# pingcap/tidb

Measured on NVIDIA H100. Metric: hash-join probe rows/sec, higher is better.
Workload: dtype int64

## Files before the change

tidb_b200/csrc/join.cu:

```cuda
#include <memory>
#include <deque>
#include <algorithm>
#include <cmath>
#include <condition_variable>
#include "join_kernels.cuh"
#include "partition_kernels.cuh"
#include "chunk_io.cuh"

namespace tg {

static const int64_t kGeneralBatchRows = 16ll << 20;
static const int64_t kDirectPushRows = 128ll << 10;
static const int64_t kNextWindowRows = 1ll << 20;

struct Side {
  int ncols = 0;
  std::vector<int> types;
  std::vector<uint32_t> flags;
  std::vector<int> elem;
  std::vector<int> kelem;
  bool has_cells = false;
  std::vector<char> needed;
  int key_col = -1;
  std::vector<int> key_cols;
// ... 664 lines not shown
  for (int c : j->build.used) if (j->build.kelem[c] != 8 || j->bcols.has_nulls[c]) return false;
  for (int e : j->kout_elem) if (e != 8) return false;
  return true;
}

static bool build_fast_out(const JoinImpl* j, const OutCols& oc, const DevCols& pview, FastOut& fo) {
  std::memset(&fo, 0, sizeof(fo));
  int pcol_of[TG_FAST_MAX_PCOLS];
  for (int c = 0; c < oc.n; c++) {
    const OutSpec& sp = oc.spec[c];
    unsigned long long* dst = reinterpret_cast<unsigned long long*>(oc.data[c]);
    if (sp.src == SRC_BUILD_KEY || (sp.src == SRC_PROBE_COL && sp.idx == j->probe.key_col)) {
      if (fo.n_key_dst >= TG_FAST_MAX_KEYDST) return false;
      fo.key_dst[fo.n_key_dst++] = dst;
    } else if (sp.src == SRC_BUILD_META) {
      if (fo.n_meta_dst >= TG_FAST_MAX_METADST) return false;
      fo.meta_dst[fo.n_meta_dst++] = dst;
    } else if (sp.src == SRC_PROBE_COL) {
      for (int q = 0; q < fo.n_pcols; q++) if (pcol_of[q] == sp.idx) return false;
      if (fo.n_pcols >= TG_FAST_MAX_PCOLS) return false;
      int k = fo.n_pcols++;
      pcol_of[k] = sp.idx;
      fo.psrc[k] = reinterpret_cast<const unsigned long long*>(pview.data[sp.idx]);
      fo.pdst[k] = dst;
    } else return false;
  }
  return true;
}

template <template <int, int, int> class F, typename... A>
static int dispatch_shape(const FastOut& fo, A&&... a) {
#define TG_SHAPE(P, K, M) if (fo.n_pcols == P && fo.n_key_dst == K && fo.n_meta_dst == M) return F<P, K, M>::run(a...);
#define TG_SHAPE_KM(P) TG_SHAPE(P, 0, 0) TG_SHAPE(P, 0, 1) TG_SHAPE(P, 1, 0) TG_SHAPE(P, 1, 1) TG_SHAPE(P, 2, 0) TG_SHAPE(P, 2, 1)
  TG_SHAPE_KM(0) TG_SHAPE_KM(1) TG_SHAPE_KM(2) TG_SHAPE_KM(3)
#undef TG_SHAPE_KM
#undef TG_SHAPE
  return fail(TG_ERR_CUDA, "internal: fused probe shape not instantiated");
}

template <int NPC, int NKD, int NMD>
struct LaunchWarp {
  static int run(JoinImpl* j, const int64_t* pkey, int64_t n, const FastOut& fo, unsigned long long* cur, const ProbeTuning& t, const SegSpec& seg) {
    constexpr int R = 4;
    static int resident = 0;
    if (!resident) {
      int nb = 0;
      if (cudaOccupancyMaxActiveBlocksPerMultiprocessor(&nb, k_probe_inner_u1_w<R, NPC, NKD, NMD>, 256, 0) != cudaSuccess || nb < 1) { cudaGetLastError(); nb = 3; }
      resident = nb;
      if (getenv("TG_DEBUG")) fprintf(stderr, "[tidbgpu] k_probe_inner_u1_w<%d,%d,%d>: %d resident CTAs per SM\n", NPC, NKD, NMD, nb);
    }
    int64_t tiles = (n + 32 * R - 1) / (32 * R);
    int64_t ctas = (tiles + 7) / 8;
    int per_sm = t.ctas_per_sm > 0 ? t.ctas_per_sm : resident;
    int grid = (int)std::min<int64_t>(ctas, (int64_t)j->nsm * per_sm);
    k_probe_inner_u1_w<R, NPC, NKD, NMD><<<grid, 256, 0, j->stream>>>(pkey, n, j->tv, fo, cur, seg);
    return TG_OK;
  }
};
template <int NPC, int NKD, int NMD>
struct LaunchSeg {
  static int run(JoinImpl* j, const int64_t* pkey, int64_t n, const FastOut& fo, unsigned long long* cur, const ProbeTuning& t, const SegSpec& seg) {
    static int resident = 0;
    if (!resident) {
      int nb = 0;
      if (cudaOccupancyMaxActiveBlocksPerMultiprocessor(&nb, k_probe_inner_u1_seg_lean<NPC, NKD, NMD>, 256, 0) != cudaSuccess || nb < 1) { cudaGetLastError(); nb = 3; }
      resident = nb;
    }
    int64_t ctas = (n / 128 + 7) / 8;
    int per_sm = t.ctas_per_sm > 0 ? t.ctas_per_sm : resident;
    int grid = (int)std::min<int64_t>(ctas, (int64_t)j->nsm * per_sm);
    k_probe_inner_u1_seg_lean<NPC, NKD, NMD><<<grid, 256, 0, j->stream>>>(pkey, n, j->tv, fo, cur, seg);
    return TG_OK;
  }
};
template <int NPC, int NKD, int NMD>
struct LaunchInplace {
  static int run(JoinImpl* j, int64_t n, const FastOut& fo, unsigned long long* cur, const ProbeTuning& t, const SegSpec& seg, uint32_t* tile_cnt) {
    if constexpr (NKD == 0) {
      return fail(TG_ERR_CUDA, "internal: the in-place segment probe needs an output fed by the join key");
    } else {
      static int resident = 0;
      if (!resident) {
        int nb = 0;
        if (cudaOccupancyMaxActiveBlocksPerMultiprocessor(&nb, k_probe_inner_u1_seg_inplace<NPC, NKD, NMD>, 256, 0) != cudaSuccess || nb < 1) { cudaGetLastError(); nb = 3; }
        resident = nb;
      }
      int64_t ctas = (n / 128 + 7) / 8;
      int per_sm = t.ctas_per_sm > 0 ? t.ctas_per_sm : resident;
      int grid = (int)std::min<int64_t>(ctas, (int64_t)j->nsm * per_sm);
      k_probe_inner_u1_seg_inplace<NPC, NKD, NMD><<<grid, 256, 0, j->stream>>>(n, j->tv, fo, cur, seg, tile_cnt);
      return TG_OK;
    }
  }
};
static int launch_probe_warp(JoinImpl* j, const int64_t* pkey, int64_t n, const FastOut& fo, unsigned long long* cur, const ProbeTuning& t,
                             const SegSpec& seg = SegSpec{nullptr, 0, 0, 0, nullptr}) {
  j->stats.paths |= TG_JOIN_PATH_PROBE_DIRECT;
  return dispatch_shape<LaunchWarp>(fo, j, pkey, n, fo, cur, t, seg);
}
static int launch_probe_seg(JoinImpl* j, const int64_t* pkey, int64_t n, const FastOut& fo, unsigned long long* cur, const ProbeTuning& t, const SegSpec& seg) {
  j->stats.paths |= TG_JOIN_PATH_PROBE_SEG;
  return dispatch_shape<LaunchSeg>(fo, j, pkey, n, fo, cur, t, seg);
}
static bool aligned16(const void* p) { return (reinterpret_cast<uintptr_t>(p) & 15) == 0; }

static int probe_device(JoinImpl* j, const DevCols& pcells, int64_t n, ResultBatch& rb, bool sync_count, const SegSpec* in_seg = nullptr) {
  const Side& p = j->probe;
  DevCols pview = pcells;
  TG_TRY(kernel_view(j, p, pview, n));
  j->stats.probe_rows += n;
  KeySpec ks = j->probe_key;
  if (j->multi_key) {
    if (in_seg) return fail(TG_ERR_UNSUPPORTED, "segmented device chunks: joins on several key columns take the general path");
    TG_TRY(composite_key(j, p, pview, n, j->pkey_syn, j->pkey_syn_nn));
    ks.data = j->pkey_syn.p; ks.nulls = j->pkey_syn_nn.as<uint8_t>();
  } else { ks.data = pview.data[p.key_col]; ks.nulls = pview.nulls[p.key_col]; }
  TG_TRY(j->out_cursor.ensure(j->device, 64));
  OutCols oc{};
  fill_outspec_probe(j, oc);
  FastOut fo{};
  const bool fast = fast_path_ok(j, pview) && build_fast_out(j, oc, pview, fo);
  if (in_seg && !fast) return fail(TG_ERR_UNSUPPORTED, "segmented device chunks are only accepted by the fused fast path (unique build keys, <= 1 payload, no filters, an output shape the warp kernels cover)");
  if (fast) {
    const ProbeTuning& tune = probe_tuning();
    const int64_t* pkey = reinterpret_cast<const int64_t*>(ks.data);
    const size_t table_bytes = (size_t)j->tv.nslots * sizeof(Slot);
    bool src16 = aligned16(pkey);
    for (int c = 0; c < fo.n_pcols; c++) src16 = src16 && aligned16(fo.psrc[c]);
    const int64_t PTILE = 1024;
    const int64_t n_main = n / PTILE * PTILE;
    int P = 0;
    int64_t C = 0;
    if (n > 0 && tune.partition && src16 && n >= (int64_t)tune.part_min_rows && table_bytes > ((size_t)tune.part_min_mb << 20)) {
      P = probe_slices(table_bytes, j->device, tune.parts);
      C = ((int64_t)((double)n_main / P * 1.05) + 16384 + 127) / 128 * 128;
      if (!(P >= 2 && (int64_t)P * C / 128 < (1ll << 31))) P = 0;
    }
    const bool inplace = P && !in_seg && rb.rows == 0 && fo.n_key_dst >= 1 &&
                         (tune.inplace >= 0 ? tune.inplace != 0 : j->seg_match >= kInplaceMinMatch);
    if (inplace) C = inplace_seg_cap(j, P, n_main, C);
    TG_TRY(ensure_result(j, rb, inplace ? std::max<int64_t>(n, (int64_t)P * C) : rb.rows + n, rb.rows > 0, rb.rows));
    for (int c = 0; c < j->n_out; c++) { oc.data[c] = kernel_out(j, rb, c) + (size_t)rb.rows * 8; oc.valid[c] = nullptr; if (rb.bitmaps[c]->p) rb.bitmaps[c]->release(); }
    build_fast_out(j, oc, pview, fo);
    unsigned long long* cur = j->out_cursor.as<unsigned long long>();
    TG_CUDA(cudaMemsetAsync(cur, 0, 8, j->stream));
    if (n > 0) {
      if (P) {
        const int nc = 1 + fo.n_pcols;
        if (!inplace) {
          for (int c = 0; c < nc; c++) {
            if (!j->part_cols[c]) j->part_cols[c].reset(new DevBuf());
            TG_TRY(j->part_cols[c]->ensure(j->device, (size_t)P * C * 8 + 64));
          }
        }
        TG_TRY(j->part_scratch.ensure(j->device, (size_t)3 * TG_MAX_PARTS * 8 + 64));
        unsigned long long* cursors = j->part_scratch.as<unsigned long long>();
        long long* bases = reinterpret_cast<long long*>(cursors + TG_MAX_PARTS);
        unsigned long long* flag = cursors + 2 * TG_MAX_PARTS;
        PartDst d{};
        d.nparts = P; d.ncols = nc;
        d.src[0] = pkey;
        for (int c = 0; c < fo.n_pcols; c++) d.src[1 + c] = fo.psrc[c];
        for (int c = 0; c < nc; c++)
          for (int q = 0; q < P; q++) d.dst[q][c] = inplace ? (c == 0 ? (void*)fo.key_dst[0] : (void*)fo.pdst[c - 1]) : j->part_cols[c]->p;
        k_segment_bases<<<1, 32, 0, j->stream>>>(cursors, bases, flag, P, C);
        d.dst_base = bases; d.capacity = C; d.overflow = flag;
        if (in_seg) { d.in_cnt = in_seg->cnt; d.in_cap = in_seg->cap; d.in_tiles_per_seg = (uint32_t)(in_seg->cap / PTILE); }
        TG_TRY(launch_partition_scatter<true>(j->device, j->stream, reinterpret_cast<const long long*>(pkey), nullptr, n_main, d, cursors,
                                              &j->stats.kernel_launches, 0, &j->stats.paths));
        const SegSpec seg{cursors, (uint32_t)(C / 128), 0, C, flag};
        if (inplace) {
          const int64_t ntiles = (int64_t)P * C / 128;
          TG_TRY(j->tile_cnt.ensure(j->device, (size_t)ntiles * 4 + 16));
          TG_TRY(j->tmp_cnt.ensure(j->device, (size_t)(2 * ntiles + 1) * 4));
          j->stats.paths |= TG_JOIN_PATH_PROBE_SEG;
          TG_TRY(dispatch_shape<LaunchInplace>(fo, j, (int64_t)P * C, fo, cur, tune, seg, j->tile_cnt.as<uint32_t>()));
          k_inplace_holes<<<grid_size(j->nsm, ntiles, 256, 4), 256, 0, j->stream>>>(j->tile_cnt.as<uint32_t>(), ntiles, cur, flag, j->tmp_cnt.as<uint32_t>());
          int64_t nblocks = 0;
          TG_TRY(enqueue_scan(j, 2 * ntiles, &nblocks));
          k_inplace_fill<<<j->nsm * 8, 256, 0, j->stream>>>(j->tile_cnt.as<uint32_t>(), ntiles, j->tmp_off.as<unsigned long long>(), cur, flag, fo);
          j->stats.kernel_launches += 3;
        } else {
          FastOut pf = fo;
          for (int c = 0; c < fo.n_pcols; c++) pf.psrc[c] = j->part_cols[1 + c]->as<unsigned long long>();
          TG_TRY(launch_probe_seg(j, j->part_cols[0]->as<int64_t>(), (int64_t)P * C, pf, cur, tune, seg));
          j->stats.kernel_launches++;
        }
        if (in_seg) TG_TRY(launch_probe_warp(j, pkey, n_main, fo, cur, tune, SegSpec{in_seg->cnt, in_seg->tiles_per_seg, 1, in_seg->cap, flag, 0}));
        else TG_TRY(launch_probe_warp(j, pkey, n, fo, cur, tune, SegSpec{nullptr, 0, 1, 0, flag, n_main < n ? n_main : 0}));
        j->stats.kernel_launches += 2;
      } else {
        if (in_seg) TG_TRY(launch_probe_warp(j, pkey, n, fo, cur, tune, SegSpec{in_seg->cnt, in_seg->tiles_per_seg, 0, in_seg->cap, nullptr}));
        else TG_TRY(launch_probe_warp(j, pkey, n, fo, cur, tune));
        j->stats.kernel_launches++;
      }
    }
    TG_TRY(gather_cells(j, rb, &pcells, cur));
    if (sync_count) {
      unsigned long long got = 0, part[2 * TG_MAX_PARTS + 1];
      const bool learn = P && !in_seg;
      if (learn) TG_CUDA(cudaMemcpyAsync(part, j->part_scratch.p, sizeof(part), cudaMemcpyDeviceToHost, j->stream));
      TG_CUDA(cudaMemcpyAsync(&got, cur, 8, cudaMemcpyDeviceToHost, j->stream));
      TG_CUDA(cudaStreamSynchronize(j->stream));
      rb.rows += (int64_t)got;
      j->stats.output_rows += (int64_t)got;
      if (P && n > 0) j->seg_match = (double)got / (double)n;
      if (learn) {
        j->seg_parts = part[2 * TG_MAX_PARTS] ? 0 : P;
        j->seg_rows = n_main;
        j->seg_fill_max = (int64_t)*std::max_element(part, part + P);
      }
    }
    return TG_OK;
  }
  if (uq_path_ok(j, pview)) {
    TG_TRY(ensure_result(j, rb, rb.rows + n, rb.rows > 0, rb.rows));
    for (int c = 0; c < j->n_out; c++) { oc.data[c] = kernel_out(j, rb, c) + (size_t)rb.rows * 8; oc.valid[c] = nullptr; if (rb.bitmaps[c]->p) rb.bitmaps[c]->release(); }
    unsigned long long* cur = j->out_cursor.as<unsigned long long>();
    TG_CUDA(cudaMemsetAsync(cur, 0, 8, j->stream));
    if (n > 0) {
      int64_t tiles = (n + 256 * UQ_R - 1) / (256 * UQ_R);
      int grid = (int)std::min<int64_t>(tiles, (int64_t)j->nsm * 8);
      k_probe_inner_uq<<<grid, 256, 0, j->stream>>>(ks, pview, p.filter, n, j->tv, oc, cur);
      j->stats.kernel_launches++;
      j->stats.paths |= TG_JOIN_PATH_PROBE_UQ;
    }
    TG_TRY(gather_cells(j, rb, &pcells, cur));
    unsigned long long got = 0;
    TG_CUDA(cudaMemcpyAsync(&got, cur, 8, cudaMemcpyDeviceToHost, j->stream));
    TG_CUDA(cudaStreamSynchronize(j->stream));
    TG_CUDA(cudaGetLastError());
    rb.rows += (int64_t)got;
    j->stats.output_rows += (int64_t)got;
    return TG_OK;
  }
  std::vector<char> nullable;
  out_nullable(j, pview, nullable);
  if ((int)j->tmp_valid.size() != j->n_out) { j->tmp_valid.clear(); for (int i = 0; i < j->n_out; i++) j->tmp_valid.emplace_back(new DevBuf()); }
  int64_t out_start = rb.rows;
  for (int64_t lo = 0; lo < n || (lo == 0 && n == 0); lo += kGeneralBatchRows) {
    int64_t m = std::min<int64_t>(kGeneralBatchRows, n - lo);
    if (m <= 0) break;
    DevCols sub = pview;
    if (lo) {
      if (lo % 8) return fail(TG_ERR_CUDA, "internal: sub-batch offset not byte aligned");
      for (int c = 0; c < p.ncols; c++) {
        if (sub.data[c]) sub.data[c] = reinterpret_cast<const uint8_t*>(sub.data[c]) + (size_t)lo * p.kelem[c];
        if (sub.nulls[c]) sub.nulls[c] += lo / 8;
      }
    }
    KeySpec sks = ks;
    if (j->multi_key) { sks.data = reinterpret_cast<const int64_t*>(ks.data) + lo; sks.nulls = ks.nulls + lo / 8; }
    else { sks.data = sub.data[p.key_col]; sks.nulls = sub.nulls[p.key_col]; }
    TG_TRY(j->tmp_cnt.ensure(j->device, (size_t)(m + 1) * 4));
    TG_TRY(j->tmp_slot.ensure(j->device, (size_t)(m + 1) * 4));
    k_probe_count<<<grid_size(j->nsm, m, 256, 8), 256, 0, j->stream>>>(sks, sub, p.filter, j->dev_other, m, j->tv, j->probe_kind, j->tmp_cnt.as<uint32_t>(),
                                                                 j->tmp_slot.as<uint32_t>(), j->need_scan ? j->slot_used.as<uint8_t>() : nullptr);
    j->stats.kernel_launches++;
    j->stats.paths |= TG_JOIN_PATH_PROBE_GENERAL;
// ... 356 lines not shown
```

tidb_b200/csrc/join_kernels.cuh:

```cuda
#pragma once
#include "common.cuh"
#include "tma.cuh"

namespace tg {

struct __align__(16) Slot { int64_t key; unsigned long long meta; };

static const uint32_t kInvalidSlot = 0xFFFFFFFFu;
static const unsigned long long kCntMask = (1ull << 28) - 1;

enum { TABLE_NONE = 0, TABLE_U1 = 1, TABLE_G = 2 };
enum { KEY_I64 = 0, KEY_F64 = 1, KEY_F32 = 2, KEY_TIME = 3 };
enum { SRC_PROBE_COL = 0, SRC_BUILD_KEY = 1, SRC_BUILD_META = 2, SRC_BUILD_WORD = 3, SRC_FLAG = 4 };

struct KeySpec {
  const void* data;
  const uint8_t* nulls;
  int32_t kind;
  int32_t reject_negative;
};

struct TableView {
  Slot* slots;
  unsigned long long nslots;
// ... 254 lines not shown
  int64_t stride = (int64_t)gridDim.x * blockDim.x;
  for (; i < n; i += stride) {
    uint32_t s = row_slot[i];
    if (s == kInvalidSlot) continue;
    unsigned long long pos = (slots[s].meta >> 28) + row_rank[i];
    unsigned long long* dst = rows + pos * rs.nwords;
    unsigned long long nullmask = 0;
    int nw = rs.null_word >= 0 ? rs.nwords - 1 : rs.nwords;
    for (int w = 0; w < nw; w++) {
      int c = rs.col[w];
      unsigned long long v;
      if (rs.elem_len[w] == 8) v = reinterpret_cast<const unsigned long long*>(cols.data[c])[i];
      else v = reinterpret_cast<const uint32_t*>(cols.data[c])[i];
      if (rs.null_bit[w] >= 0 && cols.nulls[c] && !bit_not_null(cols.nulls[c], i)) nullmask |= 1ull << rs.null_bit[w];
      dst[w] = v;
    }
    if (rs.null_word >= 0) dst[rs.null_word] = nullmask;
  }
}

#define TG_FAST_MAX_PCOLS 3
#define TG_FAST_MAX_KEYDST 2
#define TG_FAST_MAX_METADST 1
struct FastOut {
  int32_t n_pcols, n_key_dst, n_meta_dst, pad;
  const unsigned long long* psrc[TG_FAST_MAX_PCOLS];
  unsigned long long* pdst[TG_FAST_MAX_PCOLS];
  unsigned long long* key_dst[TG_FAST_MAX_KEYDST];
  unsigned long long* meta_dst[TG_FAST_MAX_METADST];
};

template <int R, int NPC, int NKD, int NMD, bool PAIRED = false>
__device__ __forceinline__ void probe_rows_u1(const int64_t (&k)[R], const unsigned long long (&pv)[R][NPC > 0 ? NPC : 1],
                                              const unsigned long long (&sl0)[R], const bool (&in)[R], const TableView& t,
                                              const FastOut& out, unsigned long long* __restrict__ out_cursor, int lane) {
  Slot v[R], w[R];
#pragma unroll
  for (int j = 0; j < R; j++) load_pair(t.slots + sl0[j], v[j], w[j]);
  unsigned bal[R];
  uint32_t total = 0;
#pragma unroll
  for (int j = 0; j < R; j++) {
    bool m;
    if (k[j] == kEmptyKey) m = in[j] && v[j].key != 0;
    else if (v[j].key == k[j]) m = true;
    else if (w[j].key == k[j]) { v[j] = w[j]; m = true; }
    else if (v[j].key == kEmptyKey || w[j].key == kEmptyKey) m = false;
    else m = probe_run(t.slots, t.nslots, k[j], sl0[j] + 2, v[j].meta);
    bal[j] = __ballot_sync(0xffffffffu, m);
    total += __popc(bal[j]);
  }
  unsigned long long wbase = 0;
  if (lane == 0 && total) wbase = atomicAdd(out_cursor, (unsigned long long)total);
  wbase = __shfl_sync(0xffffffffu, wbase, 0);
  if (PAIRED && total == 32u * R && (wbase & 1ull) == 0) {
#pragma unroll
    for (int g = 0; g < R / 2; g++) {
      const unsigned long long o = wbase + (unsigned long long)(g * 64 + 2 * lane);
      const ulonglong2 kk = make_ulonglong2((unsigned long long)k[2 * g], (unsigned long long)k[2 * g + 1]);
#pragma unroll
      for (int d = 0; d < NKD; d++) __stcs(reinterpret_cast<ulonglong2*>(out.key_dst[d] + o), kk);
#pragma unroll
      for (int d = 0; d < NMD; d++) __stcs(reinterpret_cast<ulonglong2*>(out.meta_dst[d] + o), make_ulonglong2(v[2 * g].meta, v[2 * g + 1].meta));
#pragma unroll
      for (int c = 0; c < NPC; c++) __stcs(reinterpret_cast<ulonglong2*>(out.pdst[c] + o), make_ulonglong2(pv[2 * g][c], pv[2 * g + 1][c]));
    }
    return;
  }
#pragma unroll
  for (int j = 0; j < R; j++) {
    if ((bal[j] >> lane) & 1u) {
      const unsigned long long o = wbase + __popc(bal[j] & ((1u << lane) - 1));
#pragma unroll
      for (int d = 0; d < NKD; d++) __stcs(out.key_dst[d] + o, (unsigned long long)k[j]);
#pragma unroll
      for (int d = 0; d < NMD; d++) __stcs(out.meta_dst[d] + o, v[j].meta);
#pragma unroll
      for (int c = 0; c < NPC; c++) __stcs(out.pdst[c] + o, pv[j][c]);
    }
    wbase += __popc(bal[j]);
  }
}

struct SegSpec {
  const unsigned long long* cnt;
  uint32_t tiles_per_seg;
  int32_t gate_want;
  long long cap;
  const unsigned long long* gate;
  long long ungated_from;
};

template <int R, int NPC, int NKD, int NMD>
__global__ void __launch_bounds__(256)
k_probe_inner_u1_w(const int64_t* __restrict__ pkey, int64_t n, TableView t, FastOut out,
                   unsigned long long* __restrict__ out_cursor, SegSpec seg) {
  const int64_t tile_rows = 32 * R;
  int64_t first_tile = 0;
  if (seg.gate && ((*seg.gate != 0ull) != (seg.gate_want != 0))) {
    if (seg.ungated_from <= 0 || seg.cnt) return;
    first_tile = seg.ungated_from / tile_rows;
  }
  const int lane = threadIdx.x & 31;
  const int64_t warps_total = (int64_t)gridDim.x * (blockDim.x >> 5);
  const int64_t warp_id = (int64_t)blockIdx.x * (blockDim.x >> 5) + (threadIdx.x >> 5);
  const int64_t ntiles = (n + tile_rows - 1) / tile_rows;
  for (int64_t tile = first_tile + warp_id; tile < ntiles; tile += warps_total) {
    const int64_t base = tile * tile_rows;
    int64_t limit = n;
    if (seg.cnt) {
      const uint32_t p = (uint32_t)tile / seg.tiles_per_seg;
      const unsigned long long c = seg.cnt[p];
      limit = (int64_t)p * seg.cap + (int64_t)(c < (unsigned long long)seg.cap ? c : (unsigned long long)seg.cap);
      if (base >= limit) continue;
    }
    int64_t k[R];
    unsigned long long pv[R][NPC > 0 ? NPC : 1];
    unsigned long long sl[R];
    bool in[R];
#pragma unroll
    for (int j = 0; j < R; j++) {
      int64_t i = base + j * 32 + lane;
      in[j] = i < limit;
      k[j] = in[j] ? __ldcs(pkey + i) : kEmptyKey;
    }
#pragma unroll
    for (int j = 0; j < R; j++) {
      int64_t i = base + j * 32 + lane;
      sl[j] = (k[j] == kEmptyKey) ? t.nslots : home_slot(hash64((uint64_t)k[j]), t.nslots);
#pragma unroll
      for (int c = 0; c < NPC; c++) pv[j][c] = in[j] ? __ldcs(out.psrc[c] + i) : 0ull;
    }
    probe_rows_u1<R, NPC, NKD, NMD>(k, pv, sl, in, t, out, out_cursor, lane);
  }
}

template <int NPC, int NKD, int NMD>
__device__ __forceinline__ void probe_tile_generic(const int64_t* __restrict__ pkey, int64_t base, int64_t limit, const TableView& t,
                                                   const FastOut& out, unsigned long long* __restrict__ out_cursor, int lane) {
  constexpr int R = 4;
  int64_t k[R];
  unsigned long long pv[R][NPC > 0 ? NPC : 1];
  unsigned long long sl[R];
  bool in[R];
#pragma unroll
  for (int g = 0; g < R / 2; g++) {
    const int64_t i = base + g * 64 + 2 * lane;
    const ulonglong2 kk = __ldcs(reinterpret_cast<const ulonglong2*>(pkey + i));
    in[2 * g] = i < limit; in[2 * g + 1] = i + 1 < limit;
    k[2 * g] = in[2 * g] ? (int64_t)kk.x : kEmptyKey;
    k[2 * g + 1] = in[2 * g + 1] ? (int64_t)kk.y : kEmptyKey;
  }
#pragma unroll
  for (int g = 0; g < R / 2; g++) {
    const int64_t i = base + g * 64 + 2 * lane;
    sl[2 * g] = (k[2 * g] == kEmptyKey) ? t.nslots : home_slot(hash64((uint64_t)k[2 * g]), t.nslots);
    sl[2 * g + 1] = (k[2 * g + 1] == kEmptyKey) ? t.nslots : home_slot(hash64((uint64_t)k[2 * g + 1]), t.nslots);
#pragma unroll
    for (int cc = 0; cc < NPC; cc++) {
      const ulonglong2 pp = __ldcs(reinterpret_cast<const ulonglong2*>(out.psrc[cc] + i));
      pv[2 * g][cc] = pp.x; pv[2 * g + 1][cc] = pp.y;
    }
  }
  probe_rows_u1<R, NPC, NKD, NMD, true>(k, pv, sl, in, t, out, out_cursor, lane);
}

// ... 34 lines not shown
    Slot v[R], w[R];
#pragma unroll
    for (int j = 0; j < R; j++) load_pair(t.slots + home_slot(hash64((uint64_t)k[j]), t.nslots), v[j], w[j]);
    unsigned long long meta[R];
    unsigned hit = 0, run = 0;
#pragma unroll
    for (int j = 0; j < R; j++) {
      meta[j] = 0;
      if (v[j].key == k[j]) { hit |= 1u << j; meta[j] = v[j].meta; }
      else if (w[j].key == k[j]) { hit |= 1u << j; meta[j] = w[j].meta; }
      else if (v[j].key != kEmptyKey && w[j].key != kEmptyKey) run |= 1u << j;
    }
    if (run) {
      uint32_t sl[R];
#pragma unroll
      for (int j = 0; j < R; j++) {
        const unsigned long long s = home_slot(hash64((uint64_t)k[j]), t.nslots) + 2;
        sl[j] = s == t.nslots ? 0u : (uint32_t)s;
      }
      do {
#pragma unroll
        for (int j = 0; j < R; j++) if ((run >> j) & 1u) load_pair(t.slots + sl[j], v[j], w[j]);
#pragma unroll
        for (int j = 0; j < R; j++) {
          if (!((run >> j) & 1u)) continue;
          if (v[j].key == k[j]) { hit |= 1u << j; meta[j] = v[j].meta; run &= ~(1u << j); }
          else if (v[j].key == kEmptyKey) run &= ~(1u << j);
          else if (w[j].key == k[j]) { hit |= 1u << j; meta[j] = w[j].meta; run &= ~(1u << j); }
          else if (w[j].key == kEmptyKey) run &= ~(1u << j);
          else { sl[j] += 2; if (sl[j] == t.nslots) sl[j] = 0; }
        }
      } while (run);
    }
    unsigned bal[R];
    uint32_t total = 0;
#pragma unroll
    for (int j = 0; j < R; j++) {
      bal[j] = __ballot_sync(0xffffffffu, (hit >> j) & 1u);
      total += __popc(bal[j]);
    }
    unsigned long long wbase = 0;
    if (lane == 0 && total) wbase = atomicAdd(out_cursor, (unsigned long long)total);
    wbase = __shfl_sync(0xffffffffu, wbase, 0);
    if (total == 128u && (wbase & 1ull) == 0) {
#pragma unroll
      for (int g = 0; g < G; g++) {
        const unsigned long long o = wbase + (unsigned long long)(g * 64 + 2 * lane);
        const ulonglong2 kk = make_ulonglong2((unsigned long long)k[2 * g], (unsigned long long)k[2 * g + 1]);
#pragma unroll
        for (int d = 0; d < NKD; d++) __stcs(reinterpret_cast<ulonglong2*>(out.key_dst[d] + o), kk);
#pragma unroll
        for (int d = 0; d < NMD; d++) __stcs(reinterpret_cast<ulonglong2*>(out.meta_dst[d] + o), make_ulonglong2(meta[2 * g], meta[2 * g + 1]));
#pragma unroll
        for (int cc = 0; cc < NPC; cc++) __stcs(reinterpret_cast<ulonglong2*>(out.pdst[cc] + o), make_ulonglong2(pv[2 * g][cc], pv[2 * g + 1][cc]));
      }
    } else {
#pragma unroll
      for (int j = 0; j < R; j++) {
        if ((bal[j] >> lane) & 1u) {
          const unsigned long long o = wbase + __popc(bal[j] & ((1u << lane) - 1));
#pragma unroll
          for (int d = 0; d < NKD; d++) __stcs(out.key_dst[d] + o, (unsigned long long)k[j]);
#pragma unroll
          for (int d = 0; d < NMD; d++) __stcs(out.meta_dst[d] + o, meta[j]);
#pragma unroll
          for (int cc = 0; cc < NPC; cc++) __stcs(out.pdst[cc] + o, pv[j][cc]);
        }
        wbase += __popc(bal[j]);
      }
    }
  }
  const int64_t nseg = ntiles / seg.tiles_per_seg;
  for (int64_t sp = warp_id; sp < nseg; sp += warps_total) {
    const unsigned long long cc = seg.cnt[sp];
    const int64_t fill = (int64_t)(cc < (unsigned long long)seg.cap ? cc : (unsigned long long)seg.cap);
    if ((fill & 127) == 0) continue;
    const int64_t base = (sp * seg.tiles_per_seg + fill / 128) * 128;
    probe_tile_generic<NPC, NKD, NMD>(pkey, base, sp * seg.cap + fill, t, out, out_cursor, lane);
  }
}


template <int NPC, int NKD, int NMD>
__device__ __forceinline__ void inplace_store(int64_t base, const int64_t (&k)[4], const unsigned long long (&meta)[4],
                                              const unsigned long long (&pv)[4][NPC > 0 ? NPC : 1], const unsigned (&bal)[4],
                                              const FastOut& out, int lane) {
  __syncwarp();
  int64_t o = base;
#pragma unroll
  for (int j = 0; j < 4; j++) {
    if ((bal[j] >> lane) & 1u) {
      const int64_t r = o + __popc(bal[j] & ((1u << lane) - 1));
#pragma unroll
      for (int d = 0; d < NKD; d++) __stcs(out.key_dst[d] + r, (unsigned long long)k[j]);
#pragma unroll
      for (int d = 0; d < NMD; d++) __stcs(out.meta_dst[d] + r, meta[j]);
#pragma unroll
      for (int c = 0; c < NPC; c++) __stcs(out.pdst[c] + r, pv[j][c]);
    }
    o += __popc(bal[j]);
  }
}

template <int NPC>
__device__ __forceinline__ void inplace_load_pv(int64_t base, const FastOut& out, unsigned long long (&pv)[4][NPC > 0 ? NPC : 1], int lane) {
#pragma unroll
  for (int g = 0; g < 2; g++) {
    const int64_t i = base + g * 64 + 2 * lane;
#pragma unroll
    for (int c = 0; c < NPC; c++) {
      const ulonglong2 pp = __ldcs(reinterpret_cast<const ulonglong2*>(out.pdst[c] + i));
      pv[2 * g][c] = pp.x; pv[2 * g + 1][c] = pp.y;
    }
  }
}

template <int NPC, int NKD, int NMD>
__device__ __forceinline__ uint32_t inplace_tile_generic(int64_t base, int64_t limit, const TableView& t, const FastOut& out, int lane) {
  constexpr int R = 4;
  int64_t k[R];
  unsigned long long pv[R][NPC > 0 ? NPC : 1], meta[R];
  bool in[R];
#pragma unroll
  for (int g = 0; g < R / 2; g++) {
    const int64_t i = base + g * 64 + 2 * lane;
    const ulonglong2 kk = __ldcs(reinterpret_cast<const ulonglong2*>(out.key_dst[0] + i));
    in[2 * g] = i < limit; in[2 * g + 1] = i + 1 < limit;
    k[2 * g] = in[2 * g] ? (int64_t)kk.x : kEmptyKey;
    k[2 * g + 1] = in[2 * g + 1] ? (int64_t)kk.y : kEmptyKey;
  }
  inplace_load_pv<NPC>(base, out, pv, lane);
  unsigned bal[R];
  uint32_t total = 0;
#pragma unroll
  for (int j = 0; j < R; j++) {
    const unsigned long long sl = (k[j] == kEmptyKey) ? t.nslots : home_slot(hash64((uint64_t)k[j]), t.nslots);
    Slot v, w;
    load_pair(t.slots + sl, v, w);
    bool m;
    meta[j] = v.meta;
    if (k[j] == kEmptyKey) m = in[j] && v.key != 0;
    else if (v.key == k[j]) m = true;
    else if (w.key == k[j]) { meta[j] = w.meta; m = true; }
    else if (v.key == kEmptyKey || w.key == kEmptyKey) m = false;
    else m = probe_run(t.slots, t.nslots, k[j], sl + 2, meta[j]);
    bal[j] = __ballot_sync(0xffffffffu, m);
    total += __popc(bal[j]);
  }
  inplace_store<NPC, NKD, NMD>(base, k, meta, pv, bal, out, lane);
  return total;
}

template <int NPC, int NKD, int NMD>
__global__ void __launch_bounds__(256, 3)
k_probe_inner_u1_seg_inplace(int64_t n, TableView t, FastOut out, unsigned long long* __restrict__ out_cursor, SegSpec seg,
                             uint32_t* __restrict__ tile_cnt) {
  static_assert(NKD >= 1, "the probe key is read from the first key destination");
  constexpr int R = 4, G = 2, NP = NPC > 0 ? NPC : 1;
  if (seg.gate && ((*seg.gate != 0ull) != (seg.gate_want != 0))) return;
  const int lane = threadIdx.x & 31;
  const int64_t warps_total = (int64_t)gridDim.x * (blockDim.x >> 5);
  const int64_t warp_id = (int64_t)blockIdx.x * (blockDim.x >> 5) + (threadIdx.x >> 5);
  const int64_t ntiles = n / 128;
  const int64_t* __restrict__ pkey = reinterpret_cast<const int64_t*>(out.key_dst[0]);
  unsigned long long kept = 0;
  for (int64_t tile = warp_id; tile < ntiles; tile += warps_total) {
    const int64_t base = tile * 128;
    const uint32_t p = (uint32_t)tile / seg.tiles_per_seg;
    const unsigned long long c = seg.cnt[p];
    const int64_t limit = (int64_t)p * seg.cap + (int64_t)(c < (unsigned long long)seg.cap ? c : (unsigned long long)seg.cap);
    uint32_t m = 0;
    if (limit - base >= 128) {
      int64_t k[R];
#pragma unroll
      for (int g = 0; g < G; g++) {
        const ulonglong2 kk = __ldcs(reinterpret_cast<const ulonglong2*>(pkey + base + g * 64 + 2 * lane));
        k[2 * g] = (int64_t)kk.x; k[2 * g + 1] = (int64_t)kk.y;
      }
      const bool sentinel = (k[0] == kEmptyKey) | (k[1] == kEmptyKey) | (k[2] == kEmptyKey) | (k[3] == kEmptyKey);
      if (__any_sync(0xffffffffu, sentinel)) {
        m = inplace_tile_generic<NPC, NKD, NMD>(base, limit, t, out, lane);
      } else {
        Slot v[R], w[R];
#pragma unroll
        for (int j = 0; j < R; j++) load_pair(t.slots + home_slot(hash64((uint64_t)k[j]), t.nslots), v[j], w[j]);
        unsigned long long meta[R];
        unsigned hit = 0, run = 0;
#pragma unroll
        for (int j = 0; j < R; j++) {
          meta[j] = 0;
          if (v[j].key == k[j]) { hit |= 1u << j; meta[j] = v[j].meta; }
          else if (w[j].key == k[j]) { hit |= 1u << j; meta[j] = w[j].meta; }
          else if (v[j].key != kEmptyKey && w[j].key != kEmptyKey) run |= 1u << j;
        }
        if (run) {
          uint32_t sl[R];
#pragma unroll
          for (int j = 0; j < R; j++) {
            const unsigned long long s = home_slot(hash64((uint64_t)k[j]), t.nslots) + 2;
            sl[j] = s == t.nslots ? 0u : (uint32_t)s;
          }
          do {
#pragma unroll
            for (int j = 0; j < R; j++) if ((run >> j) & 1u) load_pair(t.slots + sl[j], v[j], w[j]);
#pragma unroll
            for (int j = 0; j < R; j++) {
              if (!((run >> j) & 1u)) continue;
              if (v[j].key == k[j]) { hit |= 1u << j; meta[j] = v[j].meta; run &= ~(1u << j); }
              else if (v[j].key == kEmptyKey) run &= ~(1u << j);
              else if (w[j].key == k[j]) { hit |= 1u << j; meta[j] = w[j].meta; run &= ~(1u << j); }
              else if (w[j].key == kEmptyKey) run &= ~(1u << j);
              else { sl[j] += 2; if (sl[j] == t.nslots) sl[j] = 0; }
            }
          } while (run);
        }
        if (__all_sync(0xffffffffu, hit == 0xFu)) {
          m = 128;
#pragma unroll
          for (int g = 0; g < G; g++) {
            const int64_t o = base + g * 64 + 2 * lane;
            const ulonglong2 kk = make_ulonglong2((unsigned long long)k[2 * g], (unsigned long long)k[2 * g + 1]);
#pragma unroll
            for (int d = 1; d < NKD; d++) __stcs(reinterpret_cast<ulonglong2*>(out.key_dst[d] + o), kk);
#pragma unroll
            for (int d = 0; d < NMD; d++) __stcs(reinterpret_cast<ulonglong2*>(out.meta_dst[d] + o), make_ulonglong2(meta[2 * g], meta[2 * g + 1]));
          }
        } else {
          unsigned long long pv[R][NP];
          inplace_load_pv<NPC>(base, out, pv, lane);
          unsigned bal[R];
#pragma unroll
          for (int j = 0; j < R; j++) {
            bal[j] = __ballot_sync(0xffffffffu, (hit >> j) & 1u);
            m += __popc(bal[j]);
          }
          inplace_store<NPC, NKD, NMD>(base, k, meta, pv, bal, out, lane);
        }
      }
    } else if (limit > base) {
      m = inplace_tile_generic<NPC, NKD, NMD>(base, limit, t, out, lane);
    }
    if (lane == 0) tile_cnt[tile] = m;
    kept += m;
  }
  if (lane == 0 && kept) atomicAdd(out_cursor, kept);
}

__global__ void __launch_bounds__(256)
k_inplace_holes(const uint32_t* __restrict__ tile_cnt, int64_t ntiles, const unsigned long long* out_cursor,
                const unsigned long long* gate, uint32_t* __restrict__ cnt) {
  if (*gate) return;
  const int64_t R = (int64_t)*out_cursor;
  for (int64_t t = blockIdx.x * (int64_t)blockDim.x + threadIdx.x; t < ntiles; t += (int64_t)gridDim.x * blockDim.x) {
    const int64_t s = t * 128, e = s + tile_cnt[t];
    cnt[t] = e < R ? (uint32_t)((s + 128 < R ? s + 128 : R) - e) : 0u;
    cnt[ntiles + t] = e > R ? (uint32_t)(e - (s > R ? s : R)) : 0u;
  }
}

__device__ __forceinline__ int64_t last_le(const unsigned long long* __restrict__ off, int64_t lo, int64_t hi, unsigned long long k) {
  while (lo < hi) {
    const int64_t mid = (lo + hi + 1) >> 1;
    if (off[mid] <= k) lo = mid; else hi = mid - 1;
  }
  return lo;
}

__global__ void __launch_bounds__(256)
k_inplace_fill(const uint32_t* __restrict__ tile_cnt, int64_t ntiles, const unsigned long long* __restrict__ off,
               const unsigned long long* out_cursor, const unsigned long long* gate, FastOut out) {
  if (*gate) return;
  const int lane = threadIdx.x & 31;
  const int64_t warps_total = (int64_t)gridDim.x * (blockDim.x >> 5);
  const int64_t warp_id = (int64_t)blockIdx.x * (blockDim.x >> 5) + (threadIdx.x >> 5);
  const int64_t R = (int64_t)*out_cursor;
  const unsigned long long holes = off[ntiles];
  if (!holes) return;
  for (int64_t t = R / 128 + warp_id; t < ntiles; t += warps_total) {
    const uint32_t c = (uint32_t)(off[ntiles + t + 1] - off[ntiles + t]);
    if (!c) continue;
    const unsigned long long k0 = off[ntiles + t] - holes;
    const int64_t first = t * 128 > R ? t * 128 : R;
    const int64_t lo = last_le(off, 0, ntiles - 1, k0), hi = last_le(off, lo, ntiles - 1, k0 + c - 1);
    for (uint32_t r = lane; r < c; r += 32) {
      const unsigned long long k = k0 + r;
      const int64_t u = last_le(off, lo, hi, k);
      const int64_t dst = u * 128 + tile_cnt[u] + (int64_t)(k - off[u]), src = first + r;
      for (int d = 0; d < out.n_key_dst; d++) out.key_dst[d][dst] = out.key_dst[d][src];
      for (int d = 0; d < out.n_meta_dst; d++) out.meta_dst[d][dst] = out.meta_dst[d][src];
      for (int c2 = 0; c2 < out.n_pcols; c2++) out.pdst[c2][dst] = out.pdst[c2][src];
    }
  }
}

__device__ __forceinline__ bool other_operand(const OtherItemDev& it, bool lhs, const DevCols& pcols, int64_t i, const unsigned long long* brow,
                                              int null_word, unsigned long long& raw) {
  const int src = lhs ? it.l_src : it.r_src, idx = lhs ? it.l_idx : it.r_idx, nbit = lhs ? it.l_null_bit : it.r_null_bit;
  if (src == OSRC_PROBE) {
    const uint8_t* nb = pcols.nulls[idx];
    if (nb && !bit_not_null(nb, i)) return false;
    raw = reinterpret_cast<const unsigned long long*>(pcols.data[idx])[i];
    return true;
  }
  if (src == OSRC_BUILD) {
    if (nbit >= 0 && ((brow[null_word] >> nbit) & 1ull)) return false;
    raw = brow[idx];
    return true;
  }
  raw = it.is_real ? (unsigned long long)__double_as_longlong(it.const_f64) : (unsigned long long)it.const_i64;
  return true;
}
__device__ __forceinline__ bool eval_other(const DevOther& o, const DevCols& pcols, int64_t i, const unsigned long long* brow, int null_word) {
  for (int q = 0; q < o.n; q++) {
    const OtherItemDev& it = o.it[q];
    unsigned long long a, b;
    if (!other_operand(it, true, pcols, i, brow, null_word, a) || !other_operand(it, false, pcols, i, brow, null_word, b)) return false;
    int r = it.is_real ? cmp_real(__longlong_as_double((long long)a), __longlong_as_double((long long)b))
                       : cmp_int((int64_t)a, it.l_unsigned != 0, (int64_t)b, it.r_unsigned != 0);
    if (!apply_cmp(it.op, r)) return false;
  }
  return true;
}

__global__ void __launch_bounds__(256)
k_probe_count(KeySpec key, DevCols pcols, DevFilter filt, DevOther oth, int64_t n, TableView t, int kind,
              uint32_t* __restrict__ row_cnt, uint32_t* __restrict__ row_slot, uint8_t* slot_used) {
  int64_t i = blockIdx.x * (int64_t)blockDim.x + threadIdx.x;
  int64_t stride = (int64_t)gridDim.x * blockDim.x;
  for (; i < n; i += stride) {
    int64_t k;
    bool valid = load_key(key, i, k);
    if (valid && filt.n) valid = eval_filter(filt, pcols, i);
    uint32_t s = kInvalidSlot;
    unsigned long long meta = 0;
    if (valid) s = table_find(t, k, &meta);
    uint32_t cnt = 0;
    if (s != kInvalidSlot) cnt = t.mode == TABLE_U1 ? 1u : (uint32_t)(meta & kCntMask);
    if (oth.n && cnt) {
      const unsigned long long roff = meta >> 28;
      uint32_t pass = 0;
      for (uint32_t r = 0; r < cnt; r++) pass += eval_other(oth, pcols, i, t.rows + (roff + r) * t.row_words, t.null_word) ? 1u : 0u;
      cnt = pass;
    }
    bool matched = cnt > 0;
    if (slot_used && matched) slot_used[s] = 1;
    uint32_t c;
    switch (kind) {
      case PK_INNER: c = cnt; break;
      case PK_PROBE_OUTER: c = matched ? cnt : 1u; break;
      case PK_SEMI: c = matched ? 1u : 0u; break;
      case PK_ANTI: c = matched ? 0u : 1u; break;
      case PK_LEFT_OUTER_SEMI: case PK_ANTI_LEFT_OUTER_SEMI: c = 1u; break;
      default: c = 0u; break;
    }
    row_cnt[i] = c;
    row_slot[i] = matched ? s : kInvalidSlot;
  }
}

#define TG_SCAN_BLOCK 256
#define TG_SCAN_ITEMS 8
__global__ void __launch_bounds__(TG_SCAN_BLOCK)
k_scan_block_sums(const uint32_t* __restrict__ in, int64_t n, unsigned long long* __restrict__ block_sums) {
  __shared__ unsigned long long s[TG_SCAN_BLOCK / 32];
  int64_t base = (int64_t)blockIdx.x * TG_SCAN_BLOCK * TG_SCAN_ITEMS;
  unsigned long long sum = 0;
#pragma unroll
  for (int j = 0; j < TG_SCAN_ITEMS; j++) {
    int64_t i = base + (int64_t)j * TG_SCAN_BLOCK + threadIdx.x;
    if (i < n) sum += in[i];
// ... 249 lines not shown
```

Baseline: 28.85 billion.

## Halve in-place probe tile to 64 rows and prefetch next tile keys

The in-place segment probe now processes 64-row tiles with two keys per lane instead of 128 rows with four, and raises the occupancy target to 5 blocks per SM while capping the grid at 4 CTAs per SM. Each warp software-prefetches the next tile's keys before probing the current one, and the payload columns are loaded lazily inside the compaction step instead of up front. The aim is to cut register pressure, raise occupancy and hide key-load latency. The cost is less memory-level parallelism per warp, twice as many tiles for the holes, scan and fill kernels to process, and a larger tile_cnt array.

```diff
diff --git a/tidb_b200/csrc/join.cu b/tidb_b200/csrc/join.cu
--- a/tidb_b200/csrc/join.cu
+++ b/tidb_b200/csrc/join.cu
@@ -770,10 +770,10 @@
       static int resident = 0;
       if (!resident) {
         int nb = 0;
-        if (cudaOccupancyMaxActiveBlocksPerMultiprocessor(&nb, k_probe_inner_u1_seg_inplace<NPC, NKD, NMD>, 256, 0) != cudaSuccess || nb < 1) { cudaGetLastError(); nb = 3; }
-        resident = nb;
+        if (cudaOccupancyMaxActiveBlocksPerMultiprocessor(&nb, k_probe_inner_u1_seg_inplace<NPC, NKD, NMD>, 256, 0) != cudaSuccess || nb < 1) { cudaGetLastError(); nb = kInplaceCtasPerSm; }
+        resident = std::min(nb, kInplaceCtasPerSm);
       }
-      int64_t ctas = (n / 128 + 7) / 8;
+      int64_t ctas = (n / kInplaceTile + 7) / 8;
       int per_sm = t.ctas_per_sm > 0 ? t.ctas_per_sm : resident;
       int grid = (int)std::min<int64_t>(ctas, (int64_t)j->nsm * per_sm);
       k_probe_inner_u1_seg_inplace<NPC, NKD, NMD><<<grid, 256, 0, j->stream>>>(n, j->tv, fo, cur, seg, tile_cnt);
@@ -858,11 +858,12 @@
                                               &j->stats.kernel_launches, 0, &j->stats.paths));
         const SegSpec seg{cursors, (uint32_t)(C / 128), 0, C, flag};
         if (inplace) {
-          const int64_t ntiles = (int64_t)P * C / 128;
+          const int64_t ntiles = (int64_t)P * C / kInplaceTile;
+          const SegSpec iseg{cursors, (uint32_t)(C / kInplaceTile), 0, C, flag};
           TG_TRY(j->tile_cnt.ensure(j->device, (size_t)ntiles * 4 + 16));
           TG_TRY(j->tmp_cnt.ensure(j->device, (size_t)(2 * ntiles + 1) * 4));
           j->stats.paths |= TG_JOIN_PATH_PROBE_SEG;
-          TG_TRY(dispatch_shape<LaunchInplace>(fo, j, (int64_t)P * C, fo, cur, tune, seg, j->tile_cnt.as<uint32_t>()));
+          TG_TRY(dispatch_shape<LaunchInplace>(fo, j, (int64_t)P * C, fo, cur, tune, iseg, j->tile_cnt.as<uint32_t>()));
           k_inplace_holes<<<grid_size(j->nsm, ntiles, 256, 4), 256, 0, j->stream>>>(j->tile_cnt.as<uint32_t>(), ntiles, cur, flag, j->tmp_cnt.as<uint32_t>());
           int64_t nblocks = 0;
           TG_TRY(enqueue_scan(j, 2 * ntiles, &nblocks));
diff --git a/tidb_b200/csrc/join_kernels.cuh b/tidb_b200/csrc/join_kernels.cuh
--- a/tidb_b200/csrc/join_kernels.cuh
+++ b/tidb_b200/csrc/join_kernels.cuh
@@ -360,6 +360,9 @@
   }
 }
 
+static constexpr int kInplaceTile = 64;
+static constexpr int kInplaceCtasPerSm = 4;
+
 struct SegSpec {
   const unsigned long long* cnt;
   uint32_t tiles_per_seg;
@@ -560,58 +563,46 @@
 
 
 template <int NPC, int NKD, int NMD>
-__device__ __forceinline__ void inplace_store(int64_t base, const int64_t (&k)[4], const unsigned long long (&meta)[4],
-                                              const unsigned long long (&pv)[4][NPC > 0 ? NPC : 1], const unsigned (&bal)[4],
-                                              const FastOut& out, int lane) {
+__device__ __forceinline__ void inplace_compact(int64_t base, const int64_t (&k)[2], const unsigned long long (&meta)[2],
+                                                const unsigned (&bal)[2], const FastOut& out, int lane) {
+  const unsigned below = (1u << lane) - 1;
+  const bool keep0 = (bal[0] >> lane) & 1u, keep1 = (bal[1] >> lane) & 1u;
+  const int64_t r0 = base + __popc(bal[0] & below), r1 = base + __popc(bal[0]) + __popc(bal[1] & below);
   __syncwarp();
-  int64_t o = base;
-#pragma unroll
-  for (int j = 0; j < 4; j++) {
-    if ((bal[j] >> lane) & 1u) {
-      const int64_t r = o + __popc(bal[j] & ((1u << lane) - 1));
-#pragma unroll
-      for (int d = 0; d < NKD; d++) __stcs(out.key_dst[d] + r, (unsigned long long)k[j]);
-#pragma unroll
-      for (int d = 0; d < NMD; d++) __stcs(out.meta_dst[d] + r, meta[j]);
-#pragma unroll
-      for (int c = 0; c < NPC; c++) __stcs(out.pdst[c] + r, pv[j][c]);
-    }
-    o += __popc(bal[j]);
-  }
-}
-
-template <int NPC>
-__device__ __forceinline__ void inplace_load_pv(int64_t base, const FastOut& out, unsigned long long (&pv)[4][NPC > 0 ? NPC : 1], int lane) {
-#pragma unroll
-  for (int g = 0; g < 2; g++) {
-    const int64_t i = base + g * 64 + 2 * lane;
-#pragma unroll
-    for (int c = 0; c < NPC; c++) {
-      const ulonglong2 pp = __ldcs(reinterpret_cast<const ulonglong2*>(out.pdst[c] + i));
-      pv[2 * g][c] = pp.x; pv[2 * g + 1][c] = pp.y;
-    }
+#pragma unroll
+  for (int d = 0; d < NKD; d++) {
+    if (keep0) __stcs(out.key_dst[d] + r0, (unsigned long long)k[0]);
+    if (keep1) __stcs(out.key_dst[d] + r1, (unsigned long long)k[1]);
+  }
+#pragma unroll
+  for (int d = 0; d < NMD; d++) {
+    if (keep0) __stcs(out.meta_dst[d] + r0, meta[0]);
+    if (keep1) __stcs(out.meta_dst[d] + r1, meta[1]);
+  }
+#pragma unroll
+  for (int c = 0; c < NPC; c++) {
+    const ulonglong2 pp = __ldcs(reinterpret_cast<const ulonglong2*>(out.pdst[c] + base + 2 * lane));
+    __syncwarp();
+    if (keep0) __stcs(out.pdst[c] + r0, pp.x);
+    if (keep1) __stcs(out.pdst[c] + r1, pp.y);
   }
 }
 
 template <int NPC, int NKD, int NMD>
-__device__ __forceinline__ uint32_t inplace_tile_generic(int64_t base, int64_t limit, const TableView& t, const FastOut& out, int lane) {
-  constexpr int R = 4;
-  int64_t k[R];
-  unsigned long long pv[R][NPC > 0 ? NPC : 1], meta[R];
-  bool in[R];
-#pragma unroll
-  for (int g = 0; g < R / 2; g++) {
-    const int64_t i = base + g * 64 + 2 * lane;
-    const ulonglong2 kk = __ldcs(reinterpret_cast<const ulonglong2*>(out.key_dst[0] + i));
-    in[2 * g] = i < limit; in[2 * g + 1] = i + 1 < limit;
-    k[2 * g] = in[2 * g] ? (int64_t)kk.x : kEmptyKey;
-    k[2 * g + 1] = in[2 * g + 1] ? (int64_t)kk.y : kEmptyKey;
-  }
-  inplace_load_pv<NPC>(base, out, pv, lane);
-  unsigned bal[R];
+__device__ __forceinline__ uint32_t inplace_tile_generic(int64_t base, int64_t limit, const int64_t (&kr)[2], const TableView& t,
+                                                         const FastOut& out, int lane) {
+  int64_t k[2];
+  unsigned long long meta[2];
+  bool in[2];
+#pragma unroll
+  for (int j = 0; j < 2; j++) {
+    in[j] = base + 2 * lane + j < limit;
+    k[j] = in[j] ? kr[j] : kEmptyKey;
+  }
+  unsigned bal[2];
   uint32_t total = 0;
 #pragma unroll
-  for (int j = 0; j < R; j++) {
+  for (int j = 0; j < 2; j++) {
     const unsigned long long sl = (k[j] == kEmptyKey) ? t.nslots : home_slot(hash64((uint64_t)k[j]), t.nslots);
     Slot v, w;
     load_pair(t.slots + sl, v, w);
@@ -625,64 +616,62 @@
     bal[j] = __ballot_sync(0xffffffffu, m);
     total += __popc(bal[j]);
   }
-  inplace_store<NPC, NKD, NMD>(base, k, meta, pv, bal, out, lane);
+  inplace_compact<NPC, NKD, NMD>(base, k, meta, bal, out, lane);
   return total;
 }
 
 template <int NPC, int NKD, int NMD>
-__global__ void __launch_bounds__(256, 3)
+__global__ void __launch_bounds__(256, 5)
 k_probe_inner_u1_seg_inplace(int64_t n, TableView t, FastOut out, unsigned long long* __restrict__ out_cursor, SegSpec seg,
                              uint32_t* __restrict__ tile_cnt) {
   static_assert(NKD >= 1, "the probe key is read from the first key destination");
-  constexpr int R = 4, G = 2, NP = NPC > 0 ? NPC : 1;
+  constexpr int T = kInplaceTile;
   if (seg.gate && ((*seg.gate != 0ull) != (seg.gate_want != 0))) return;
   const int lane = threadIdx.x & 31;
-  const int64_t warps_total = (int64_t)gridDim.x * (blockDim.x >> 5);
-  const int64_t warp_id = (int64_t)blockIdx.x * (blockDim.x >> 5) + (threadIdx.x >> 5);
-  const int64_t ntiles = n / 128;
-  const int64_t* __restrict__ pkey = reinterpret_cast<const int64_t*>(out.key_dst[0]);
+  const uint32_t warps_total = gridDim.x * (blockDim.x >> 5);
+  const uint32_t warp_id = blockIdx.x * (blockDim.x >> 5) + (threadIdx.x >> 5);
+  const uint32_t ntiles = (uint32_t)(n / T);
+  const int64_t* __restrict__ pkey = reinterpret_cast<const int64_t*>(out.key_dst[0]) + 2 * lane;
   unsigned long long kept = 0;
-  for (int64_t tile = warp_id; tile < ntiles; tile += warps_total) {
-    const int64_t base = tile * 128;
-    const uint32_t p = (uint32_t)tile / seg.tiles_per_seg;
+  ulonglong2 nk = make_ulonglong2(0ull, 0ull);
+  if (warp_id < ntiles) nk = __ldcs(reinterpret_cast<const ulonglong2*>(pkey + (int64_t)warp_id * T));
+  for (uint32_t tile = warp_id; tile < ntiles; tile += warps_total) {
+    const int64_t k[2] = {(int64_t)nk.x, (int64_t)nk.y};
+    const uint32_t next = tile + warps_total;
+    if (next < ntiles) nk = __ldcs(reinterpret_cast<const ulonglong2*>(pkey + (int64_t)next * T));
+    const int64_t base = (int64_t)tile * T;
+    const uint32_t p = tile / seg.tiles_per_seg;
     const unsigned long long c = seg.cnt[p];
     const int64_t limit = (int64_t)p * seg.cap + (int64_t)(c < (unsigned long long)seg.cap ? c : (unsigned long long)seg.cap);
     uint32_t m = 0;
-    if (limit - base >= 128) {
-      int64_t k[R];
-#pragma unroll
-      for (int g = 0; g < G; g++) {
-        const ulonglong2 kk = __ldcs(reinterpret_cast<const ulonglong2*>(pkey + base + g * 64 + 2 * lane));
-        k[2 * g] = (int64_t)kk.x; k[2 * g + 1] = (int64_t)kk.y;
-      }
-      const bool sentinel = (k[0] == kEmptyKey) | (k[1] == kEmptyKey) | (k[2] == kEmptyKey) | (k[3] == kEmptyKey);
-      if (__any_sync(0xffffffffu, sentinel)) {
-        m = inplace_tile_generic<NPC, NKD, NMD>(base, limit, t, out, lane);
+    if (limit - base >= T) {
+      if (__any_sync(0xffffffffu, (k[0] == kEmptyKey) | (k[1] == kEmptyKey))) {
+        m = inplace_tile_generic<NPC, NKD, NMD>(base, limit, k, t, out, lane);
       } else {
-        Slot v[R], w[R];
-#pragma unroll
-        for (int j = 0; j < R; j++) load_pair(t.slots + home_slot(hash64((uint64_t)k[j]), t.nslots), v[j], w[j]);
-        unsigned long long meta[R];
+        Slot v[2], w[2];
+#pragma unroll
+        for (int j = 0; j < 2; j++) load_pair(t.slots + home_slot(hash64((uint64_t)k[j]), t.nslots), v[j], w[j]);
+        unsigned long long meta[2];
         unsigned hit = 0, run = 0;
 #pragma unroll
-        for (int j = 0; j < R; j++) {
+        for (int j = 0; j < 2; j++) {
           meta[j] = 0;
           if (v[j].key == k[j]) { hit |= 1u << j; meta[j] = v[j].meta; }
           else if (w[j].key == k[j]) { hit |= 1u << j; meta[j] = w[j].meta; }
           else if (v[j].key != kEmptyKey && w[j].key != kEmptyKey) run |= 1u << j;
         }
         if (run) {
-          uint32_t sl[R];
-#pragma unroll
-          for (int j = 0; j < R; j++) {
+          uint32_t sl[2];
+#pragma unroll
+          for (int j = 0; j < 2; j++) {
             const unsigned long long s = home_slot(hash64((uint64_t)k[j]), t.nslots) + 2;
             sl[j] = s == t.nslots ? 0u : (uint32_t)s;
           }
           do {
 #pragma unroll
-            for (int j = 0; j < R; j++) if ((run >> j) & 1u) load_pair(t.slots + sl[j], v[j], w[j]);
-#pragma unroll
-            for (int j = 0; j < R; j++) {
+            for (int j = 0; j < 2; j++) if ((run >> j) & 1u) load_pair(t.slots + sl[j], v[j], w[j]);
+#pragma unroll
+            for (int j = 0; j < 2; j++) {
               if (!((run >> j) & 1u)) continue;
               if (v[j].key == k[j]) { hit |= 1u << j; meta[j] = v[j].meta; run &= ~(1u << j); }
               else if (v[j].key == kEmptyKey) run &= ~(1u << j);
@@ -692,31 +681,26 @@
             }
           } while (run);
         }
-        if (__all_sync(0xffffffffu, hit == 0xFu)) {
-          m = 128;
-#pragma unroll
-          for (int g = 0; g < G; g++) {
-            const int64_t o = base + g * 64 + 2 * lane;
-            const ulonglong2 kk = make_ulonglong2((unsigned long long)k[2 * g], (unsigned long long)k[2 * g + 1]);
-#pragma unroll
-            for (int d = 1; d < NKD; d++) __stcs(reinterpret_cast<ulonglong2*>(out.key_dst[d] + o), kk);
-#pragma unroll
-            for (int d = 0; d < NMD; d++) __stcs(reinterpret_cast<ulonglong2*>(out.meta_dst[d] + o), make_ulonglong2(meta[2 * g], meta[2 * g + 1]));
-          }
+        if (__all_sync(0xffffffffu, hit == 3u)) {
+          m = T;
+          const int64_t o = base + 2 * lane;
+          const ulonglong2 kk = make_ulonglong2((unsigned long long)k[0], (unsigned long long)k[1]);
+#pragma unroll
+          for (int d = 1; d < NKD; d++) __stcs(reinterpret_cast<ulonglong2*>(out.key_dst[d] + o), kk);
+#pragma unroll
+          for (int d = 0; d < NMD; d++) __stcs(reinterpret_cast<ulonglong2*>(out.meta_dst[d] + o), make_ulonglong2(meta[0], meta[1]));
         } else {
-          unsigned long long pv[R][NP];
-          inplace_load_pv<NPC>(base, out, pv, lane);
-          unsigned bal[R];
-#pragma unroll
-          for (int j = 0; j < R; j++) {
+          unsigned bal[2];
+#pragma unroll
+          for (int j = 0; j < 2; j++) {
             bal[j] = __ballot_sync(0xffffffffu, (hit >> j) & 1u);
             m += __popc(bal[j]);
           }
-          inplace_store<NPC, NKD, NMD>(base, k, meta, pv, bal, out, lane);
+          inplace_compact<NPC, NKD, NMD>(base, k, meta, bal, out, lane);
         }
       }
     } else if (limit > base) {
-      m = inplace_tile_generic<NPC, NKD, NMD>(base, limit, t, out, lane);
+      m = inplace_tile_generic<NPC, NKD, NMD>(base, limit, k, t, out, lane);
     }
     if (lane == 0) tile_cnt[tile] = m;
     kept += m;
@@ -727,11 +711,12 @@
 __global__ void __launch_bounds__(256)
 k_inplace_holes(const uint32_t* __restrict__ tile_cnt, int64_t ntiles, const unsigned long long* out_cursor,
                 const unsigned long long* gate, uint32_t* __restrict__ cnt) {
+  constexpr int64_t T = kInplaceTile;
   if (*gate) return;
   const int64_t R = (int64_t)*out_cursor;
   for (int64_t t = blockIdx.x * (int64_t)blockDim.x + threadIdx.x; t < ntiles; t += (int64_t)gridDim.x * blockDim.x) {
-    const int64_t s = t * 128, e = s + tile_cnt[t];
-    cnt[t] = e < R ? (uint32_t)((s + 128 < R ? s + 128 : R) - e) : 0u;
+    const int64_t s = t * T, e = s + tile_cnt[t];
+    cnt[t] = e < R ? (uint32_t)((s + T < R ? s + T : R) - e) : 0u;
     cnt[ntiles + t] = e > R ? (uint32_t)(e - (s > R ? s : R)) : 0u;
   }
 }
@@ -747,6 +732,7 @@
 __global__ void __launch_bounds__(256)
 k_inplace_fill(const uint32_t* __restrict__ tile_cnt, int64_t ntiles, const unsigned long long* __restrict__ off,
                const unsigned long long* out_cursor, const unsigned long long* gate, FastOut out) {
+  constexpr int64_t T = kInplaceTile;
   if (*gate) return;
   const int lane = threadIdx.x & 31;
   const int64_t warps_total = (int64_t)gridDim.x * (blockDim.x >> 5);
@@ -754,16 +740,16 @@
   const int64_t R = (int64_t)*out_cursor;
   const unsigned long long holes = off[ntiles];
   if (!holes) return;
-  for (int64_t t = R / 128 + warp_id; t < ntiles; t += warps_total) {
+  for (int64_t t = R / T + warp_id; t < ntiles; t += warps_total) {
     const uint32_t c = (uint32_t)(off[ntiles + t + 1] - off[ntiles + t]);
     if (!c) continue;
     const unsigned long long k0 = off[ntiles + t] - holes;
-    const int64_t first = t * 128 > R ? t * 128 : R;
+    const int64_t first = t * T > R ? t * T : R;
     const int64_t lo = last_le(off, 0, ntiles - 1, k0), hi = last_le(off, lo, ntiles - 1, k0 + c - 1);
     for (uint32_t r = lane; r < c; r += 32) {
       const unsigned long long k = k0 + r;
       const int64_t u = last_le(off, lo, hi, k);
-      const int64_t dst = u * 128 + tile_cnt[u] + (int64_t)(k - off[u]), src = first + r;
+      const int64_t dst = u * T + tile_cnt[u] + (int64_t)(k - off[u]), src = first + r;
       for (int d = 0; d < out.n_key_dst; d++) out.key_dst[d][dst] = out.key_dst[d][src];
       for (int d = 0; d < out.n_meta_dst; d++) out.meta_dst[d][dst] = out.meta_dst[d][src];
       for (int c2 = 0; c2 < out.n_pcols; c2++) out.pdst[c2][dst] = out.pdst[c2][src];
```

Measured after the change: 29.15 billion (median of 6 runs). +1.1%, better.
